# facebookresearch/co-tracker

Hardware: NVIDIA B200
Metric: tracked points*frames/sec at N=6400, T=16, 512^2 (higher is better)
Workload: dtype transformer + corr_mlp.fc2 + input_transform: bf16x3; correlation einsum: fp16x2; corr_mlp.fc1: bf16x3; fp32 accumulate, fp32 softmax/LayerNorm/GELU

## Files before the change

### cotracker_b200/csrc/api.cu

```cuda
#include <stdio.h>
#include <string.h>

#include <atomic>
#include <string>
#include <vector>

#include "../../include/ct3_b200.h"
#include "gemm.cuh"
#include "kernels.cuh"

using namespace ct3;

namespace {

thread_local char g_err[512] = "";
struct OptDef { const char* name; int lo, hi; };
enum { OPT_GEMM = 0, OPT_CORR, OPT_ATTN, OPT_PREC_CORR, OPT_PREC_FC1, OPT_FUSE, OPT_COUNT };
constexpr int kDefPrecCorr = 2, kDefPrecFc1 = 3;
constexpr OptDef kOptDefs[OPT_COUNT] = {
    {"gemm", 0, 1},
    {"corr", 0, 3},
    {"attn", 0, 2},
    {"prec.corr", 1, 3},
    {"prec.fc1", 1, 3},
    {"fuse", 0, 2},
};
thread_local int g_opt[OPT_COUNT] = {0, 0, 0, kDefPrecCorr, kDefPrecFc1, 1};
#define g_opt_gemm g_opt[OPT_GEMM]
#define g_opt_corr g_opt[OPT_CORR]
#define g_opt_attn g_opt[OPT_ATTN]

int fail(int code, const char* fmt, const char* detail = "") {
  snprintf(g_err, sizeof(g_err), fmt, detail);
  return code;
}
int fail_cuda(cudaError_t e, const char* where) {
  snprintf(g_err, sizeof(g_err), "%s: %s", where, cudaGetErrorString(e));
  return CT3_ECUDA;
}
#define CK(call, where)                                  \
  do {                                                   \
    cudaError_t e__ = (call);                            \
    if (e__ != cudaSuccess) return fail_cuda(e__, where); \
  } while (0)

int num_sms() {
  static std::atomic<int> cache[64] = {};
  int dev = 0;
  if (cudaGetDevice(&dev) != cudaSuccess) return 148;
  if (dev >= 0 && dev < 64) {
    const int c = cache[dev].load(std::memory_order_relaxed);
    if (c > 0) return c;
  }
  int n = 0;
  if (cudaDeviceGetAttribute(&n, cudaDevAttrMultiProcessorCount, dev) != cudaSuccess || n <= 0) n = 148;
  if (dev >= 0 && dev < 64) cache[dev].store(n, std::memory_order_relaxed);
  return n;
}


enum { CAT_CORR = 0, CAT_GEMM = 1, CAT_ATTN = 2, CAT_LN = 3, CAT_MISC = 4, CAT_ENC = 5, CAT_QKVA = 6, CAT_COUNT = 7 };
struct ProfRec { int cat; cudaEvent_t a, b; double flops; int launches; };
thread_local bool g_prof_on = false;
thread_local std::vector<ProfRec> g_prof;
struct ProfScope {
  cudaStream_t s; int cat; double flops; int launches; cudaEvent_t a = nullptr, b = nullptr;
  ProfScope(cudaStream_t s_, int cat_, double flops_ = 0.0, int launches_ = 1)
      : s(s_), cat(cat_), flops(flops_), launches(launches_) {
    if (g_prof_on && cat_ >= 0) { cudaEventCreate(&a); cudaEventCreate(&b); cudaEventRecord(a, s); }
  }
  ~ProfScope() {
    if (a) { cudaEventRecord(b, s); g_prof.push_back({cat, a, b, flops, launches}); }
  }
};

size_t align_up(size_t x, size_t a = 256) { return (x + a - 1) / a * a; }

struct Lin {
  size_t w = 0, b = 0;
  size_t ws = 0;
  int N = 0, K = 0, Kpad = 0;
};
struct Block {
  Lin qkv_h;
  Lin q;
  Lin kv;
  Lin kv_f;
  Lin out, fc1, fc2;
  size_t ctx_g = 0, ctx_b = 0;
  bool cross = false;
};
struct Layout {
  Lin corr_fc1, corr_fc2, in_tr;
  Lin corr_fc1_h;
  Lin corr_fc1_t, corr_fc1_th;
  Block time[kDepth], vself[kDepth], p2v[kDepth], v2p[kDepth];
  size_t heads_w = 0, heads_b = 0, virt = 0, win_f32 = 0;
  size_t scratch = 0;
  size_t total = 0;
};

int pad64(int k) { return (k + 63) / 64 * 64; }

void place_lin(Lin& l, int N, int K, size_t& off) {
  l.N = N;
  l.K = K;
  l.Kpad = pad64(K);
  l.w = off;
  off = align_up(off + (size_t)N * 2 * l.Kpad * sizeof(__nv_bfloat16));
  l.b = off;
// ... 88 lines not shown
  float* att_part;
  __nv_bfloat16* pyr_split;
  size_t total;
};
Workspace carve(void* base, int T, int N, int H4 = 0, int W4 = 0) {
  Workspace w;
  const size_t R = (size_t)(N + kV) * T, Rp = (size_t)N * T, Rv = (size_t)kV * T, Mc = Rp * kL;
  uint8_t* p = reinterpret_cast<uint8_t*>(base);
  size_t off = 0;
  auto take = [&](size_t bytes) { uint8_t* r = p + off; off = align_up(off + bytes, 1024); return r; };
  w.vol = (__nv_bfloat16*)take(Mc * 2 * kVolPad * 2);
  w.h1 = (__nv_bfloat16*)take(Mc * 2 * kCorrHid * 2);
  w.xs = (__nv_bfloat16*)take(Rp * 2 * kXPad * 2);
  w.tokens = (float*)take(R * kC * 4);
  w.traw = (__nv_bfloat16*)take(R * 2 * kC * 2);
  w.tstat = (float*)take(R * kLnParts * 2 * 4);
  w.ln = (__nv_bfloat16*)take(R * 2 * kC * 2);
  w.att = (__nv_bfloat16*)take(R * 2 * kC * 2);
  w.qkv = (float*)take(R * 3 * kC * 4);
  w.vqkv = (float*)take(Rv * 3 * kC * 4);
  w.hmid = (__nv_bfloat16*)take(R * 2 * kMlpHid * 2);
  w.row_bias = (float*)take((size_t)T * kC * 4);
  w.att_part = (float*)take(attention_partial_bytes(T, kV, kAttnMaxSplits));
  w.pyr_split = nullptr;
  if (H4 > 0 && W4 > 0 && corr_patch_supported(T, H4, W4))
    w.pyr_split = (__nv_bfloat16*)take((size_t)pyramid_layout(T, H4, W4).total * 4);
  w.total = off;
  return w;
}

struct Runner {
  const uint8_t* pk;
  const Layout& L;
  cudaStream_t s;
  int impl;
  const char* gerr = nullptr;

  int gemm(const __nv_bfloat16* x, const Lin& lin, int M, const GemmEpilogue& e, int products = 3, int fp16 = 0,
           int64_t x_ld = 0) {
    GemmProblem p;
    p.products = products;
    p.fp16 = fp16;
    p.x_ld = x_ld;
    p.x_split = x;
    p.w_split = reinterpret_cast<const __nv_bfloat16*>(pk + lin.w);
    p.M = M;
    p.N = lin.N;
    p.Kpad = lin.Kpad;
    p.epi = e;
    if (!p.epi.bias) p.epi.bias = reinterpret_cast<const float*>(pk + lin.b);
    if (M == 0) return 0;
    ProfScope ps(s, CAT_GEMM, 2.0 * (double)M * lin.N * lin.K);
    return gemm_launch(p, impl, num_sms(), s, &gerr);
  }
  static GemmEpilogue to_f32(float* out, int ld, bool residual) {
    GemmEpilogue e;
    e.out_f32 = out; e.ld_f32 = ld; e.residual = residual ? 1 : 0;
    return e;
  }
  static GemmEpilogue to_split(__nv_bfloat16* out, int ld, int lo_off, int act) {
    GemmEpilogue e;
    e.out_split = out; e.ld_split = ld; e.lo_off = lo_off; e.act = act;
    return e;
  }
};

#define RUNC(cat, call)                                                                  \
  do {                                                                                   \
    int rc__;                                                                            \
    { ProfScope ps__(R.s, cat); rc__ = (int)(call); }                                    \
    if (rc__ != 0) {                                                                     \
      snprintf(g_err, sizeof(g_err), "%s failed: %s (%s)", #call,                        \
               cudaGetErrorString((cudaError_t)rc__), R.gerr ? R.gerr : "");             \
      return CT3_ECUDA;                                                                  \
    }                                                                                    \
  } while (0)

int run_attention(Runner& R, const Workspace& W, const AttnParams& a, bool per_warp) {
  if (g_opt_attn == 1) return (int)launch_attention(a, R.s);
  if (g_opt_attn == 0 && !per_warp && a.Lq > kV && attention_p2v_supported(a)) return (int)launch_attention_p2v(a, R.s);
  return (int)launch_attention_tc(a, per_warp, W.att_part, num_sms(), R.s);
}

int mlp_half(Runner& R, const Workspace& W, const Block& b, int64_t row0, int rows) {
  float* x = W.tokens + row0 * kC;
  __nv_bfloat16* ln = W.ln + row0 * 2 * kC;
  __nv_bfloat16* hm = W.hmid + row0 * 2 * kMlpHid;
  RUNC(CAT_LN, launch_layernorm_split(x, rows, nullptr, nullptr, 1e-6f, ln, R.s));
  RUNC(-1, R.gemm(ln, b.fc1, rows, Runner::to_split(hm, 2 * kMlpHid, kMlpHid,  2)));
  RUNC(-1, R.gemm(hm, b.fc2, rows, Runner::to_f32(x, kC, true)));
  return 0;
}

int transformer_body(Runner& R, const Workspace& W, int T, int N) {
  const Layout& L = R.L;
  const int Rp = N * T, Rv = kV * T, Rall = Rp + Rv;
  const float scale = 1.0f / sqrtf((float)kDh);
  const uint8_t* pk = R.pk;
  RUNC(CAT_MISC, launch_init_virtual(W.tokens, reinterpret_cast<const float*>(pk + L.virt), T, N, R.s));
  float* vtok = W.tokens + (int64_t)Rp * kC;
  __nv_bfloat16* ln_p = W.ln;
  __nv_bfloat16* ln_v = W.ln + (int64_t)Rp * 2 * kC;
  __nv_bfloat16* att_p = W.att;
  __nv_bfloat16* att_v = W.att + (int64_t)Rp * 2 * kC;

  for (int i = 0; i < kDepth; ++i) {
    {
      const Block& b = L.time[i];
      RUNC(CAT_LN, launch_layernorm_split(W.tokens, Rall, nullptr, nullptr, 1e-6f, W.ln, R.s));
      if (g_opt[OPT_FUSE] >= 1 && R.impl == 0 && g_opt_attn != 1 && qkv_time_attn_supported(T)) {
        ProfScope ps(R.s, CAT_QKVA, 0.0);
        int rc = gemm_qkv_time_attn_launch(W.ln, reinterpret_cast<const __nv_bfloat16*>(pk + b.qkv_h.w),
                                           reinterpret_cast<const float*>(pk + b.qkv_h.b), Rall, kC, T, W.att, 2 * kC,
                                           kC, scale, nullptr, nullptr, 0.f, num_sms(), R.s, &R.gerr);
        if (rc != 0) {
          snprintf(g_err, sizeof(g_err), "fused qkv + time attention failed: %s (%s)",
                   cudaGetErrorString((cudaError_t)rc), R.gerr ? R.gerr : "");
          return CT3_ECUDA;
        }
      } else {
        RUNC(-1, R.gemm(W.ln, b.q, Rall, Runner::to_f32(W.qkv, 3 * kC, false)));
        AttnParams a{};
        a.q = W.qkv; a.q_ld = 3 * kC; a.q_col = 0;
        a.kv = W.qkv; a.kv_ld = 3 * kC; a.k_col = kC; a.v_col = 2 * kC;
        a.out = W.att; a.out_ld = 2 * kC; a.lo_off = kC;
        a.num_seq = N + kV; a.Lq = T; a.Lk = T;
        a.q_seq_stride = T; a.q_tok_stride = 1; a.k_seq_stride = T; a.k_tok_stride = 1;
        a.scale = scale;
        RUNC(CAT_ATTN, run_attention(R, W, a, true));
      }
      RUNC(-1, R.gemm(W.att, b.out, Rall, Runner::to_f32(W.tokens, kC, true)));
      if (int rc = mlp_half(R, W, b, 0, Rall)) return rc;
    }
    {
      const Block& b = L.v2p[i];
      RUNC(CAT_LN, launch_layernorm_split(vtok, Rv, nullptr, nullptr, 1e-6f, ln_v, R.s));
      RUNC(CAT_LN, launch_layernorm_split(W.tokens, Rp, reinterpret_cast<const float*>(pk + b.ctx_g),
                                 reinterpret_cast<const float*>(pk + b.ctx_b), 1e-5f, ln_p, R.s));
      RUNC(-1, R.gemm(ln_v, b.q, Rv, Runner::to_f32(W.vqkv, kC, false)));
      RUNC(-1, R.gemm(ln_p, b.kv, Rp, Runner::to_f32(W.qkv, 2 * kC, false)));
      AttnParams a{};
      a.q = W.vqkv; a.q_ld = kC; a.q_col = 0;
      a.kv = W.qkv; a.kv_ld = 2 * kC; a.k_col = 0; a.v_col = kC;
      a.out = att_v; a.out_ld = 2 * kC; a.lo_off = kC;
      a.num_seq = T; a.Lq = kV; a.Lk = N;
      a.q_seq_stride = 1; a.q_tok_stride = T; a.k_seq_stride = 1; a.k_tok_stride = T;
      a.scale = scale;
      RUNC(CAT_ATTN, run_attention(R, W, a, false));
      RUNC(-1, R.gemm(att_v, b.out, Rv, Runner::to_f32(vtok, kC, true)));
      if (int rc = mlp_half(R, W, b, Rp, Rv)) return rc;
    }
    {
      const Block& b = L.vself[i];
      RUNC(CAT_LN, launch_layernorm_split(vtok, Rv, nullptr, nullptr, 1e-6f, ln_v, R.s));
      RUNC(-1, R.gemm(ln_v, b.q, Rv, Runner::to_f32(W.vqkv, 3 * kC, false)));
      AttnParams a{};
      a.q = W.vqkv; a.q_ld = 3 * kC; a.q_col = 0;
      a.kv = W.vqkv; a.kv_ld = 3 * kC; a.k_col = kC; a.v_col = 2 * kC;
      a.out = att_v; a.out_ld = 2 * kC; a.lo_off = kC;
      a.num_seq = T; a.Lq = kV; a.Lk = kV;
      a.q_seq_stride = 1; a.q_tok_stride = T; a.k_seq_stride = 1; a.k_tok_stride = T;
      a.scale = scale;
      RUNC(CAT_ATTN, run_attention(R, W, a, false));
      RUNC(-1, R.gemm(att_v, b.out, Rv, Runner::to_f32(vtok, kC, true)));
      if (int rc = mlp_half(R, W, b, Rp, Rv)) return rc;
    }
    {
      const Block& b = L.p2v[i];
      RUNC(CAT_LN, launch_layernorm_split(W.tokens, Rp, nullptr, nullptr, 1e-6f, ln_p, R.s));
      RUNC(CAT_LN, launch_layernorm_split(vtok, Rv, reinterpret_cast<const float*>(pk + b.ctx_g),
                                 reinterpret_cast<const float*>(pk + b.ctx_b), 1e-5f, ln_v, R.s));
// ... 838 lines not shown
```

### cotracker_b200/csrc/common.cuh

```cuda
#pragma once
#include <cuda.h>
#include <cuda_bf16.h>
#include <cuda_fp16.h>
#include <cuda_runtime.h>
#include <stdint.h>

#include <atomic>

namespace ct3 {

struct DeviceOnce { std::atomic<uint64_t> done[2] = {}; };
template <typename F>
inline cudaError_t once_per_device(DeviceOnce& flag, F&& f) {
  int dev = 0;
  cudaError_t e = cudaGetDevice(&dev);
  if (e != cudaSuccess) return e;
  if (dev < 0 || dev >= 128) return f();
  const uint64_t bit = 1ull << (dev & 63);
  if (flag.done[dev >> 6].load(std::memory_order_acquire) & bit) return cudaSuccess;
  e = f();
  if (e == cudaSuccess) flag.done[dev >> 6].fetch_or(bit, std::memory_order_release);
  return e;
}

// ... 245 lines not shown
  asm volatile("tcgen05.dealloc.cta_group::1.sync.aligned.b32 %0, %1;" ::"r"(taddr), "r"(ncols) : "memory");
}
__device__ __forceinline__ uint64_t umma_desc_sw128(uint32_t smem_addr) {
  uint64_t d = 0;
  d |= (uint64_t)((smem_addr & 0x3FFFFu) >> 4);
  d |= (uint64_t)1 << 16;
  d |= (uint64_t)(1024 >> 4) << 32;
  d |= (uint64_t)1 << 46;
  d |= (uint64_t)2 << 61;
  return d;
}
__host__ __device__ constexpr uint32_t umma_idesc_bf16(int M, int N) {
  return (1u << 4) | (1u << 7) | (1u << 10) | ((uint32_t)(N >> 3) << 17) | ((uint32_t)(M >> 4) << 24);
}
__host__ __device__ constexpr uint32_t umma_idesc_16(int M, int N, bool fp16) {
  return (1u << 4) | (fp16 ? 0u : ((1u << 7) | (1u << 10))) | ((uint32_t)(N >> 3) << 17) | ((uint32_t)(M >> 4) << 24);
}
__device__ __forceinline__ void umma_bf16(uint32_t d_tmem, uint64_t adesc, uint64_t bdesc, uint32_t idesc,
                                          uint32_t accumulate) {
  asm volatile(
      "{\n\t"
      ".reg .pred p;\n\t"
      "setp.ne.b32 p, %4, 0;\n\t"
      "tcgen05.mma.cta_group::1.kind::f16 [%0], %1, %2, %3, p;\n\t"
      "}" ::"r"(d_tmem),
      "l"(adesc), "l"(bdesc), "r"(idesc), "r"(accumulate)
      : "memory");
}
__device__ __forceinline__ void umma_commit(uint64_t* bar) {
  asm volatile("tcgen05.commit.cta_group::1.mbarrier::arrive::one.shared::cluster.b64 [%0];" ::"r"(smem_u32(bar))
               : "memory");
}
__device__ __forceinline__ void umma_commit_mc(uint64_t* bar, uint16_t mask) {
  asm volatile(
      "tcgen05.commit.cta_group::1.mbarrier::arrive::one.shared::cluster.multicast::cluster.b64 [%0], %1;" ::"r"(
          smem_u32(bar)),
      "h"(mask)
      : "memory");
}
constexpr uint32_t kPeerBitMask = 0xFEFFFFFFu;
__device__ __forceinline__ void tmem_alloc_2sm(uint32_t* dst_smem, uint32_t ncols) {
  asm volatile("tcgen05.alloc.cta_group::2.sync.aligned.shared::cta.b32 [%0], %1;" ::"r"(smem_u32(dst_smem)),
               "r"(ncols)
               : "memory");
  asm volatile("tcgen05.relinquish_alloc_permit.cta_group::2.sync.aligned;" ::: "memory");
}
__device__ __forceinline__ void tmem_dealloc_2sm(uint32_t taddr, uint32_t ncols) {
  asm volatile("tcgen05.dealloc.cta_group::2.sync.aligned.b32 %0, %1;" ::"r"(taddr), "r"(ncols) : "memory");
}
__device__ __forceinline__ void tma_load_2d_2sm(void* smem_dst, const CUtensorMap* m, int c0, int c1, uint64_t* bar) {
  asm volatile(
      "cp.async.bulk.tensor.2d.cta_group::2.shared::cluster.global.mbarrier::complete_tx::bytes [%0], [%1, {%3, %4}], [%2];"
      ::"r"(smem_u32(smem_dst)), "l"(reinterpret_cast<uint64_t>(m)), "r"(smem_u32(bar) & kPeerBitMask), "r"(c0), "r"(c1)
      : "memory");
}
__device__ __forceinline__ void umma_bf16_2sm(uint32_t d_tmem, uint64_t adesc, uint64_t bdesc, uint32_t idesc,
                                              uint32_t accumulate) {
  asm volatile(
      "{\n\t"
      ".reg .pred p;\n\t"
      "setp.ne.b32 p, %4, 0;\n\t"
      "tcgen05.mma.cta_group::2.kind::f16 [%0], %1, %2, %3, p;\n\t"
      "}" ::"r"(d_tmem),
      "l"(adesc), "l"(bdesc), "r"(idesc), "r"(accumulate)
      : "memory");
}
__device__ __forceinline__ void umma_commit_2sm(uint64_t* bar) {
  asm volatile(
      "tcgen05.commit.cta_group::2.mbarrier::arrive::one.shared::cluster.multicast::cluster.b64 [%0], %1;" ::"r"(
          smem_u32(bar)),
      "h"((uint16_t)3)
      : "memory");
}
__device__ __forceinline__ void mbar_arrive_remote(uint64_t* bar, uint32_t cta) {
  asm volatile(
      "{\n\t"
      ".reg .b32 ra;\n\t"
      "mapa.shared::cluster.u32 ra, %0, %1;\n\t"
      "mbarrier.arrive.shared::cluster.b64 _, [ra];\n\t"
      "}" ::"r"(smem_u32(bar)),
      "r"(cta)
      : "memory");
}
__device__ __forceinline__ void tmem_ld32(uint32_t taddr, float (&v)[32]) {
  uint32_t r[32];
  asm volatile(
      "tcgen05.ld.sync.aligned.32x32b.x32.b32 "
      "{%0, %1, %2, %3, %4, %5, %6, %7, %8, %9, %10, %11, %12, %13, %14, %15, "
      "%16, %17, %18, %19, %20, %21, %22, %23, %24, %25, %26, %27, %28, %29, %30, %31}, [%32];"
      : "=r"(r[0]), "=r"(r[1]), "=r"(r[2]), "=r"(r[3]), "=r"(r[4]), "=r"(r[5]), "=r"(r[6]), "=r"(r[7]),
        "=r"(r[8]), "=r"(r[9]), "=r"(r[10]), "=r"(r[11]), "=r"(r[12]), "=r"(r[13]), "=r"(r[14]), "=r"(r[15]),
        "=r"(r[16]), "=r"(r[17]), "=r"(r[18]), "=r"(r[19]), "=r"(r[20]), "=r"(r[21]), "=r"(r[22]), "=r"(r[23]),
        "=r"(r[24]), "=r"(r[25]), "=r"(r[26]), "=r"(r[27]), "=r"(r[28]), "=r"(r[29]), "=r"(r[30]), "=r"(r[31])
      : "r"(taddr)
      : "memory");
  asm volatile("tcgen05.wait::ld.sync.aligned;" : "+r"(r[0]), "+r"(r[1]), "+r"(r[2]), "+r"(r[3]), "+r"(r[4]), "+r"(r[5]), "+r"(r[6]), "+r"(r[7]), "+r"(r[8]), "+r"(r[9]), "+r"(r[10]), "+r"(r[11]), "+r"(r[12]), "+r"(r[13]), "+r"(r[14]), "+r"(r[15]), "+r"(r[16]), "+r"(r[17]), "+r"(r[18]), "+r"(r[19]), "+r"(r[20]), "+r"(r[21]), "+r"(r[22]), "+r"(r[23]), "+r"(r[24]), "+r"(r[25]), "+r"(r[26]), "+r"(r[27]), "+r"(r[28]), "+r"(r[29]), "+r"(r[30]), "+r"(r[31]) :: "memory");
#pragma unroll
  for (int i = 0; i < 32; ++i) v[i] = __uint_as_float(r[i]);
}

__device__ __forceinline__ void tmem_ld8_nowait(uint32_t taddr, uint32_t (&r)[8]) {
  asm volatile(
      "tcgen05.ld.sync.aligned.32x32b.x8.b32 {%0, %1, %2, %3, %4, %5, %6, %7}, [%8];"
      : "=r"(r[0]), "=r"(r[1]), "=r"(r[2]), "=r"(r[3]), "=r"(r[4]), "=r"(r[5]), "=r"(r[6]), "=r"(r[7])
      : "r"(taddr)
      : "memory");
}
__device__ __forceinline__ void tmem_ld_wait() { asm volatile("tcgen05.wait::ld.sync.aligned;" ::: "memory"); }
__device__ __forceinline__ void tmem_ld_wait8(uint32_t (&r)[8]) {
  asm volatile("tcgen05.wait::ld.sync.aligned;"
               : "+r"(r[0]), "+r"(r[1]), "+r"(r[2]), "+r"(r[3]), "+r"(r[4]), "+r"(r[5]), "+r"(r[6]), "+r"(r[7])
               ::"memory");
}

__device__ __forceinline__ void tmem_ld64(uint32_t taddr, float (&v)[64]) {
  uint32_t r[64];
  asm volatile(
      "tcgen05.ld.sync.aligned.32x32b.x64.b32 "
      "{%0, %1, %2, %3, %4, %5, %6, %7, %8, %9, %10, %11, %12, %13, %14, %15, %16, %17, %18, %19, %20, %21, %22, %23, %24, %25, %26, %27, %28, %29, %30, %31, %32, %33, %34, %35, %36, %37, %38, %39, %40, %41, %42, %43, %44, %45, %46, %47, %48, %49, %50, %51, %52, %53, %54, %55, %56, %57, %58, %59, %60, %61, %62, %63}, [%64];"
      : "=r"(r[0]), "=r"(r[1]), "=r"(r[2]), "=r"(r[3]), "=r"(r[4]), "=r"(r[5]), "=r"(r[6]), "=r"(r[7]), "=r"(r[8]), "=r"(r[9]), "=r"(r[10]), "=r"(r[11]), "=r"(r[12]), "=r"(r[13]), "=r"(r[14]), "=r"(r[15]), "=r"(r[16]), "=r"(r[17]), "=r"(r[18]), "=r"(r[19]), "=r"(r[20]), "=r"(r[21]), "=r"(r[22]), "=r"(r[23]), "=r"(r[24]), "=r"(r[25]), "=r"(r[26]), "=r"(r[27]), "=r"(r[28]), "=r"(r[29]), "=r"(r[30]), "=r"(r[31]), "=r"(r[32]), "=r"(r[33]), "=r"(r[34]), "=r"(r[35]), "=r"(r[36]), "=r"(r[37]), "=r"(r[38]), "=r"(r[39]), "=r"(r[40]), "=r"(r[41]), "=r"(r[42]), "=r"(r[43]), "=r"(r[44]), "=r"(r[45]), "=r"(r[46]), "=r"(r[47]), "=r"(r[48]), "=r"(r[49]), "=r"(r[50]), "=r"(r[51]), "=r"(r[52]), "=r"(r[53]), "=r"(r[54]), "=r"(r[55]), "=r"(r[56]), "=r"(r[57]), "=r"(r[58]), "=r"(r[59]), "=r"(r[60]), "=r"(r[61]), "=r"(r[62]), "=r"(r[63])
      : "r"(taddr)
      : "memory");
  asm volatile("tcgen05.wait::ld.sync.aligned;"
               : "+r"(r[0]), "+r"(r[1]), "+r"(r[2]), "+r"(r[3]), "+r"(r[4]), "+r"(r[5]), "+r"(r[6]), "+r"(r[7]), "+r"(r[8]), "+r"(r[9]), "+r"(r[10]), "+r"(r[11]), "+r"(r[12]), "+r"(r[13]), "+r"(r[14]), "+r"(r[15]), "+r"(r[16]), "+r"(r[17]), "+r"(r[18]), "+r"(r[19]), "+r"(r[20]), "+r"(r[21]), "+r"(r[22]), "+r"(r[23]), "+r"(r[24]), "+r"(r[25]), "+r"(r[26]), "+r"(r[27]), "+r"(r[28]), "+r"(r[29]), "+r"(r[30]), "+r"(r[31]), "+r"(r[32]), "+r"(r[33]), "+r"(r[34]), "+r"(r[35]), "+r"(r[36]), "+r"(r[37]), "+r"(r[38]), "+r"(r[39]), "+r"(r[40]), "+r"(r[41]), "+r"(r[42]), "+r"(r[43]), "+r"(r[44]), "+r"(r[45]), "+r"(r[46]), "+r"(r[47]), "+r"(r[48]), "+r"(r[49]), "+r"(r[50]), "+r"(r[51]), "+r"(r[52]), "+r"(r[53]), "+r"(r[54]), "+r"(r[55]), "+r"(r[56]), "+r"(r[57]), "+r"(r[58]), "+r"(r[59]), "+r"(r[60]), "+r"(r[61]), "+r"(r[62]), "+r"(r[63])
               ::"memory");
#pragma unroll
  for (int i = 0; i < 64; ++i) v[i] = __uint_as_float(r[i]);
}

__device__ __forceinline__ void tmem_ld16(uint32_t taddr, float (&v)[16]) {
  uint32_t r[16];
  asm volatile(
      "tcgen05.ld.sync.aligned.32x32b.x16.b32 "
      "{%0, %1, %2, %3, %4, %5, %6, %7, %8, %9, %10, %11, %12, %13, %14, %15}, [%16];"
      : "=r"(r[0]), "=r"(r[1]), "=r"(r[2]), "=r"(r[3]), "=r"(r[4]), "=r"(r[5]), "=r"(r[6]), "=r"(r[7]),
        "=r"(r[8]), "=r"(r[9]), "=r"(r[10]), "=r"(r[11]), "=r"(r[12]), "=r"(r[13]), "=r"(r[14]), "=r"(r[15])
      : "r"(taddr)
      : "memory");
  asm volatile("tcgen05.wait::ld.sync.aligned;"
               : "+r"(r[0]), "+r"(r[1]), "+r"(r[2]), "+r"(r[3]), "+r"(r[4]), "+r"(r[5]), "+r"(r[6]), "+r"(r[7]),
                 "+r"(r[8]), "+r"(r[9]), "+r"(r[10]), "+r"(r[11]), "+r"(r[12]), "+r"(r[13]), "+r"(r[14]), "+r"(r[15])
               ::"memory");
#pragma unroll
  for (int i = 0; i < 16; ++i) v[i] = __uint_as_float(r[i]);
}

}
```

### cotracker_b200/csrc/gemm.cu

```cuda
#include "gemm.cuh"

namespace ct3 {
namespace {

constexpr int BM = 128, BN = 128, BK = 64;
constexpr int ACC = 2;
constexpr int TILE_A = BM * BK * 2;
constexpr int TILE_B = BN * BK * 2;
constexpr int EPI_WARPS = 16;
constexpr int CW = 16;
constexpr int STG_WORDS = 32 * CW;
constexpr int MAX_STAGES = 6;
template <int NPROD>
struct Cfg {
  static constexpr int AP = NPROD >= 3 ? 2 : 1;
  static constexpr int BP = NPROD >= 2 ? 2 : 1;
  static constexpr int STAGE_BYTES = AP * TILE_A + BP * TILE_B;
  static constexpr int STAGES = NPROD >= 3 ? 3 : (NPROD == 2 ? 4 : 6);
  static constexpr int OFF_B = AP * TILE_A;
};
constexpr int OFF_STG = 3 * 65536;
static_assert(Cfg<1>::STAGES * Cfg<1>::STAGE_BYTES == OFF_STG && Cfg<2>::STAGES * Cfg<2>::STAGE_BYTES == OFF_STG &&
              Cfg<3>::STAGES * Cfg<3>::STAGE_BYTES == OFF_STG && Cfg<4>::STAGES * Cfg<4>::STAGE_BYTES == OFF_STG &&
              Cfg<5>::STAGES * Cfg<5>::STAGE_BYTES == OFF_STG, "ring size");
// ... 303 lines not shown
        for (int kb = 0; kb < num_kb; ++kb) {
          mbar_wait(&empty_bar[stage], phase ^ 1u);
          if (rank == 0) mbar_arrive_expect_tx(&full_bar[stage], TX_BYTES);
          uint8_t* s = smem + stage * STAGE_BYTES;
          tma_load_2d_2sm(s, &tmX, kb * BK, mt * BM, &full_bar[stage]);
          if (C::AP == 2) tma_load_2d_2sm(s + TILE_A, &tmX, Kpad + kb * BK, mt * BM, &full_bar[stage]);
          tma_load_2d_2sm(s + C::OFF_B, &tmW, kb * BK, wrow, &full_bar[stage]);
          if (C::BP == 2) tma_load_2d_2sm(s + C::OFF_B + TILE_B, &tmW, Kpad + kb * BK, wrow, &full_bar[stage]);
          if (++stage == STAGES) { stage = 0; phase ^= 1u; }
        }
      }
    }
  } else if (warp == 1) {
    if (rank == 0 && elect_one()) {
      const uint32_t idesc = umma_idesc_16(256, BNP, fp16 != 0);
      int stage = 0, acc = 0;
      uint32_t phase = 0, acc_phase = 0;
      for (int tile = first; tile < num_tiles; tile += step) {
        mbar_wait(&tempty_bar[acc], acc_phase ^ 1u);
        tc_fence_after_sync();
        const uint32_t d_tmem = tmem_base + (uint32_t)(acc * BNP);
        for (int kb = 0; kb < num_kb; ++kb) {
          mbar_wait(&full_bar[stage], phase);
          tc_fence_after_sync();
          const uint32_t s = smem_u32(smem + stage * STAGE_BYTES);
          const uint32_t a_hi = s, a_lo = s + TILE_A, b_hi = s + C::OFF_B, b_lo = b_hi + TILE_B;
#pragma unroll
          for (int kk = 0; kk < BK / 16; ++kk) {
            const uint32_t koff = kk * 32;
            const uint64_t dah = umma_desc_sw128(a_hi + koff), dbh = umma_desc_sw128(b_hi + koff);
            const uint32_t first = (kb | kk) != 0 ? 1u : 0u;
            if (NPROD >= 3) {
              umma_bf16_2sm(d_tmem, umma_desc_sw128(a_lo + koff), dbh, idesc, first);
              umma_bf16_2sm(d_tmem, dah, umma_desc_sw128(b_lo + koff), idesc, 1u);
              umma_bf16_2sm(d_tmem, dah, dbh, idesc, 1u);
            } else if (NPROD == 2) {
              umma_bf16_2sm(d_tmem, dah, umma_desc_sw128(b_lo + koff), idesc, first);
              umma_bf16_2sm(d_tmem, dah, dbh, idesc, 1u);
            } else {
              umma_bf16_2sm(d_tmem, dah, dbh, idesc, first);
            }
          }
          umma_commit_2sm(&empty_bar[stage]);
          if (++stage == STAGES) { stage = 0; phase ^= 1u; }
        }
        umma_commit_2sm(&tfull_bar[acc]);
        if (++acc == ACC) { acc = 0; acc_phase ^= 1u; }
      }
    }
  } else {
    const int quarter = warp & 3;
    constexpr int CH = BNP / CW / (EPI_WARPS / 4);
    const int chunk0 = ((warp - 2) >> 2) * CH;
    int acc = 0;
    uint32_t acc_phase = 0;
    for (int tile = first; tile < num_tiles; tile += step) {
      const int mt = (tile / num_nt) * 2 + (int)rank, nt = tile % num_nt;
      mbar_wait(&tfull_bar[acc], acc_phase);
      tc_fence_after_sync();
      const int row0 = mt * BM + quarter * 32;
      uint32_t* stg = reinterpret_cast<uint32_t*>(smem + OFF_STG) + (warp - 2) * STG_WORDS;
      float ln_mean = 0.f, ln_rstd = 1.f;
      if constexpr (NPROD == 5) {
        if (row0 + lane < M) ln_row_stats(epi.ln_part + (int64_t)(row0 + lane) * kLnParts * 2, epi.ln_eps, ln_mean, ln_rstd);
      }
#pragma unroll 1
      for (int chunk = chunk0; chunk < chunk0 + CH; ++chunk) {
        float v[CW];
        const uint32_t taddr = tmem_base + ((uint32_t)(quarter * 32) << 16) + (uint32_t)(acc * BNP + chunk * CW);
        tmem_ld16(taddr, v);
        epilogue_chunk<NPROD == 4, NPROD == 5>(epi, M, N, row0, nt * BNP + chunk * CW, lane, v, stg, ln_mean, ln_rstd);
      }
      tc_fence_before_sync();
      __syncwarp();
      if (lane == 0) mbar_arrive_remote(&tempty_bar[acc], 0);
      if (++acc == ACC) { acc = 0; acc_phase ^= 1u; }
    }
  }

  tc_fence_before_sync();
  __syncthreads();
  cluster_sync_all();
  if (warp == 1) tmem_dealloc_2sm(tmem_base, TCOLS);
}

namespace qa {
constexpr int BNQ = 144;
constexpr int TILE_BQ = (BNQ / 2) * BK * 2;
constexpr int STAGE = 2 * TILE_A + 2 * TILE_BQ;
constexpr int NSTAGE = 2;
constexpr int KV_LD = 100;
constexpr int KV_BYTES = BM * KV_LD * 4;
constexpr int OFF_KV = NSTAGE * STAGE;
constexpr int OFF_BARQ = OFF_KV + 2 * KV_BYTES;
constexpr int SMEM = OFF_BARQ + 256 + 1024;
constexpr int EPIW = 8;
constexpr int NTHREADS = (2 + EPIW) * 32;
constexpr int ACC_STRIDE = 256;
static_assert(SMEM <= 232448, "shared memory budget");
}

__global__ void __launch_bounds__(qa::NTHREADS, 1)
gemm_qkv_time_attn_kernel(const __grid_constant__ CUtensorMap tmX, const __grid_constant__ CUtensorMap tmW, int M,
                          int Kpad, int T, int R, float scale_log2e, GemmEpilogue epi) {
  using namespace qa;
  constexpr uint32_t TX_BYTES = 2u * (2u * TILE_A + 2u * TILE_BQ);
  extern __shared__ __align__(1024) uint8_t smem_raw[];
  uint8_t* smem = smem_align1024(smem_raw);
  uint64_t* full_bar = reinterpret_cast<uint64_t*>(smem + OFF_BARQ);
  uint64_t* empty_bar = full_bar + NSTAGE;
  uint64_t* tfull_bar = empty_bar + NSTAGE;
  uint64_t* tempty_bar = tfull_bar + ACC;
  uint32_t* tmem_slot = reinterpret_cast<uint32_t*>(tempty_bar + ACC);
  float* kvs = reinterpret_cast<float*>(smem + OFF_KV);

  const int warp = threadIdx.x >> 5, lane = threadIdx.x & 31;
  const uint32_t rank = cluster_ctarank();
  if (warp == 0 && lane == 0) {
    tma_prefetch_desc(&tmX);
    tma_prefetch_desc(&tmW);
    for (int i = 0; i < NSTAGE; ++i) {
      mbar_init(&full_bar[i], 1);
      mbar_init(&empty_bar[i], 1);
    }
    for (int i = 0; i < ACC; ++i) {
      mbar_init(&tfull_bar[i], 1);
      mbar_init(&tempty_bar[i], 2 * 4);
    }
    fence_barrier_init();
  }
  if (warp == 1) tmem_alloc_2sm(tmem_slot, 512);
  tc_fence_before_sync();
  __syncthreads();
  cluster_sync_all();
  tc_fence_after_sync();
  const uint32_t tmem_base = *tmem_slot;

  const int num_mt = (M + R - 1) / R;
  const int num_mp = (num_mt + 1) / 2;
  const int num_tiles = num_mp * kHeads;
  const int num_kb = Kpad / BK;
  const int first = blockIdx.x >> 1, step = gridDim.x >> 1;

  if (warp == 0) {
    if (elect_one()) {
      int stage = 0;
      uint32_t phase = 0;
      for (int tile = first; tile < num_tiles; tile += step) {
        const int mt = (tile / kHeads) * 2 + (int)rank, h = tile % kHeads;
        const int wrow = h * BNQ + (int)rank * (BNQ / 2);
        for (int kb = 0; kb < num_kb; ++kb) {
          mbar_wait(&empty_bar[stage], phase ^ 1u);
          if (rank == 0) mbar_arrive_expect_tx(&full_bar[stage], TX_BYTES);
          uint8_t* s = smem + stage * STAGE;
          tma_load_2d_2sm(s, &tmX, kb * BK, mt * R, &full_bar[stage]);
          tma_load_2d_2sm(s + TILE_A, &tmX, Kpad + kb * BK, mt * R, &full_bar[stage]);
          tma_load_2d_2sm(s + 2 * TILE_A, &tmW, kb * BK, wrow, &full_bar[stage]);
          tma_load_2d_2sm(s + 2 * TILE_A + TILE_BQ, &tmW, Kpad + kb * BK, wrow, &full_bar[stage]);
          if (++stage == NSTAGE) { stage = 0; phase ^= 1u; }
        }
      }
    }
  } else if (warp == 1) {
    if (rank == 0 && elect_one()) {
      constexpr uint32_t idesc = umma_idesc_bf16(256, BNQ);
      int stage = 0, acc = 0;
// ... 286 lines not shown
  }
  const int groups = ((num_mt + 1) / 2) * (p.N / bnp);
  int pairs = num_sms / 2;
  if (pairs > groups) pairs = groups;
  cudaLaunchConfig_t cfg = {};
  cfg.gridDim = dim3(2 * pairs);
  cfg.blockDim = dim3(THREADS);
  cfg.dynamicSmemBytes = SMEM_BYTES;
  cfg.stream = stream;
  cudaLaunchAttribute at[1];
  at[0].id = cudaLaunchAttributeClusterDimension;
  at[0].val.clusterDim.x = 2;
  at[0].val.clusterDim.y = 1;
  at[0].val.clusterDim.z = 1;
  cfg.attrs = at;
  cfg.numAttrs = 1;
  cudaError_t e = (bnp == 256)
      ? cudaLaunchKernelEx(&cfg, gemm_split3_pair_kernel<256, NPROD>, tmX, tmW, p.M, p.N, p.Kpad, p.fp16, p.epi)
      : cudaLaunchKernelEx(&cfg, gemm_split3_pair_kernel<192, NPROD>, tmX, tmW, p.M, p.N, p.Kpad, p.fp16, p.epi);
  if (e != cudaSuccess) return e;
  return cudaGetLastError();
}

}

bool qkv_time_attn_supported(int T) { return T >= 1 && T <= BM; }

int gemm_qkv_time_attn_launch(const __nv_bfloat16* x_split, const __nv_bfloat16* w_heads, const float* bias_heads,
                              int M, int Kpad, int T, __nv_bfloat16* att_split, int64_t ld_split, int lo_off,
                              float scale, const float* ln_part, const float* ln_wsum, float ln_eps, int num_sms,
                              cudaStream_t stream, const char** err) {
  *err = nullptr;
  if (M <= 0 || Kpad <= 0 || (Kpad % BK) != 0 || !qkv_time_attn_supported(T) || (M % T) != 0) {
    *err = "qkv_time_attn: need M > 0, M % T == 0, 1 <= T <= 128, Kpad % 64 == 0";
    return (int)cudaErrorInvalidValue;
  }
  if (((reinterpret_cast<uintptr_t>(x_split) | reinterpret_cast<uintptr_t>(w_heads) |
        reinterpret_cast<uintptr_t>(att_split)) & 15) || (ld_split % 8) != 0 || (lo_off % 8) != 0) {
    *err = "qkv_time_attn: operands must be 16-byte aligned";
    return (int)cudaErrorInvalidValue;
  }
  const int R = (BM / T) * T;
  CUtensorMap tmX, tmW;
  if (!make_tmap(&tmX, x_split, (uint64_t)M, 2ull * Kpad) ||
      !make_tmap(&tmW, w_heads, (uint64_t)(kHeads * qa::BNQ), 2ull * Kpad, (uint32_t)(qa::BNQ / 2))) {
    *err = "qkv_time_attn: cuTensorMapEncodeTiled failed";
    return (int)cudaErrorInvalidValue;
  }
  static DeviceOnce attr;
  cudaError_t e = once_per_device(attr, [&] {
    return cudaFuncSetAttribute(gemm_qkv_time_attn_kernel, cudaFuncAttributeMaxDynamicSharedMemorySize, qa::SMEM);
  });
  if (e != cudaSuccess) { *err = "qkv_time_attn: cudaFuncSetAttribute failed"; return (int)e; }
  const int num_mt = (M + R - 1) / R;
  const int groups = ((num_mt + 1) / 2) * kHeads;
  int pairs = num_sms / 2;
  if (pairs > groups) pairs = groups;
  GemmEpilogue epi;
  epi.bias = bias_heads;
  epi.out_split = att_split;
  epi.ld_split = ld_split;
  epi.lo_off = lo_off;
  epi.ln_part = ln_part;
  epi.ln_wsum = ln_wsum;
  epi.ln_eps = ln_eps;
  cudaLaunchConfig_t cfg = {};
  cfg.gridDim = dim3(2 * pairs);
  cfg.blockDim = dim3(qa::NTHREADS);
  cfg.dynamicSmemBytes = qa::SMEM;
  cfg.stream = stream;
  cudaLaunchAttribute at[1];
  at[0].id = cudaLaunchAttributeClusterDimension;
  at[0].val.clusterDim.x = 2;
  at[0].val.clusterDim.y = 1;
  at[0].val.clusterDim.z = 1;
  cfg.attrs = at;
  cfg.numAttrs = 1;
  e = cudaLaunchKernelEx(&cfg, gemm_qkv_time_attn_kernel, tmX, tmW, M, Kpad, T, R,
                         scale * 1.44269504088896340736f, epi);
  if (e != cudaSuccess) return (int)e;
  return (int)cudaGetLastError();
}

int gemm_launch(const GemmProblem& p, int impl, int num_sms, cudaStream_t stream, const char** err) {
  *err = nullptr;
  if (p.M <= 0 || p.N <= 0 || p.Kpad <= 0 || (p.N % BN) != 0 || (p.Kpad % BK) != 0) {
    *err = "gemm: need M>0, N % 128 == 0, Kpad % 64 == 0";
    return (int)cudaErrorInvalidValue;
  }
  if (p.products < 1 || p.products > 3) {
    *err = "gemm: products must be 1, 2 or 3";
    return (int)cudaErrorInvalidValue;
  }
  const int64_t x_ld = p.x_ld ? p.x_ld : 2 * (int64_t)p.Kpad;
  if (x_ld < (p.products == 3 ? 2 : 1) * (int64_t)p.Kpad || (x_ld % 8) != 0) {
    *err = "gemm: x_ld too small for the operand planes this product count reads";
    return (int)cudaErrorInvalidValue;
  }
  if ((reinterpret_cast<uintptr_t>(p.x_split) | reinterpret_cast<uintptr_t>(p.w_split)) & 15) {
    *err = "gemm: operands must be 16-byte aligned";
    return (int)cudaErrorInvalidValue;
  }
  if (p.epi.raw_split && (p.N != kLnDim || !p.epi.out_f32 || !p.epi.stat_part || impl == 1)) {
    *err = "gemm: raw_split/stat_part need the fp32 output path of the tensor-core kernels with N == 384";
    return (int)cudaErrorInvalidValue;
  }
  if (p.epi.ln_part && !p.epi.ln_wsum) {
    *err = "gemm: ln_part needs ln_wsum";
    return (int)cudaErrorInvalidValue;
  }
  if (impl == 1) {
    dim3 grid((p.N + 63) / 64, (p.M + 63) / 64);
    gemm_split3_simt_kernel<<<grid, 256, 0, stream>>>(p.x_split, p.w_split, p.M, p.N, p.Kpad, x_ld, p.products,
                                                      p.fp16, p.epi);
    return (int)cudaGetLastError();
  }
  const int num_mt = (p.M + BM - 1) / BM;
  int bnp = 0;
  if (impl == 0 && num_mt >= 2 * num_sms) bnp = (p.N % 256 == 0) ? 256 : ((p.N % 192 == 0) ? 192 : 0);
  CUtensorMap tmX, tmW;
  if (!make_tmap(&tmX, p.x_split, (uint64_t)p.M, (uint64_t)x_ld) ||
      !make_tmap(&tmW, p.w_split, (uint64_t)p.N, 2ull * p.Kpad, bnp ? (uint32_t)(bnp / 2) : 128u)) {
    *err = "gemm: cuTensorMapEncodeTiled failed";
    return (int)cudaErrorInvalidValue;
  }
  static DeviceOnce attr_set;
  {
    cudaError_t e = once_per_device(attr_set, [&] {
      cudaError_t e = set_attrs<3>();
      if (e == cudaSuccess) e = set_attrs<4>();
      if (e == cudaSuccess) e = set_attrs<5>();
      if (e == cudaSuccess) e = set_attrs<2>();
      if (e == cudaSuccess) e = set_attrs<1>();
      return e;
    });
    if (e != cudaSuccess) { *err = "gemm: cudaFuncSetAttribute(max dynamic smem) failed"; return (int)e; }
  }
  if (p.epi.ln_part && (p.products != 3 || p.epi.raw_split)) {
    *err = "gemm: the LayerNorm-consumer epilogue needs 3 products and cannot be combined with raw_split";
    return (int)cudaErrorInvalidValue;
  }
  cudaError_t e = (p.products == 3 && p.epi.raw_split) ? launch_tc<4>(p, tmX, tmW, bnp, num_mt, num_sms, stream)
                : (p.products == 3 && p.epi.ln_part) ? launch_tc<5>(p, tmX, tmW, bnp, num_mt, num_sms, stream)
                : p.products == 3 ? launch_tc<3>(p, tmX, tmW, bnp, num_mt, num_sms, stream)
                : p.products == 2 ? launch_tc<2>(p, tmX, tmW, bnp, num_mt, num_sms, stream)
                                  : launch_tc<1>(p, tmX, tmW, bnp, num_mt, num_sms, stream);
  return (int)e;
}

}
```

### cotracker_b200/csrc/gemm.cuh

```cuda
#pragma once
#include "common.cuh"

namespace ct3 {

struct GemmEpilogue {
  const float* bias = nullptr;
  const float* row_bias = nullptr;
  int row_mod = 1;
  int act = 0;
  float* out_f32 = nullptr;
  int64_t ld_f32 = 0;
  int residual = 0;
  __nv_bfloat16* out_split = nullptr;
  int64_t ld_split = 0;
  int lo_off = 0;
  int row_group = 1;
  const float* ln_part = nullptr;
  const float* ln_wsum = nullptr;
  float ln_eps = 0.f;
  __nv_bfloat16* raw_split = nullptr;
  float* stat_part = nullptr;
};
constexpr int kLnDim = 384;
constexpr int kLnParts = kLnDim / 16;

struct GemmProblem {
  const __nv_bfloat16* x_split;
  const __nv_bfloat16* w_split;
  int M, N, Kpad;
  int products = 3;
  int fp16 = 0;
  int64_t x_ld = 0;
  GemmEpilogue epi;
};

bool encode_tensor_map(CUtensorMap* m, CUtensorMapDataType dtype, int rank, const void* base, const uint64_t* dims,
                       const uint64_t* strides_bytes, const uint32_t* box, CUtensorMapSwizzle swizzle);

int gemm_launch(const GemmProblem& p, int impl, int num_sms, cudaStream_t stream, const char** err);

bool qkv_time_attn_supported(int T);
int gemm_qkv_time_attn_launch(const __nv_bfloat16* x_split, const __nv_bfloat16* w_heads, const float* bias_heads,
                              int M, int Kpad, int T, __nv_bfloat16* att_split, int64_t ld_split, int lo_off,
                              float scale, const float* ln_part, const float* ln_wsum, float ln_eps, int num_sms,
                              cudaStream_t stream, const char** err);

__device__ __forceinline__ void ln_row_stats(const float* part, float eps, float& mean, float& rstd) {
  float s = 0.f, ss = 0.f;
#pragma unroll
  for (int i = 0; i < kLnParts; ++i) {
    const float2 p = __ldg(reinterpret_cast<const float2*>(part) + i);
    s += p.x;
    ss += p.y;
  }
  mean = s * (1.0f / kLnDim);
  const float var = fmaxf(ss * (1.0f / kLnDim) - mean * mean, 0.f);
  rstd = rsqrtf(var + eps);
}

}
```

Before: 1.195 million.

## Fuse transformer MLP fc1, GELU and fc2 into one 2-SM tcgen05 kernel

Adds a persistent 2-CTA cluster kernel that computes fc1 per 128-wide hidden chunk into TMEM, applies bias, GELU and a bf16 hi/lo split into shared memory, then feeds that chunk directly into the fc2 accumulation with the residual epilogue. This removes the round trip of the 1536-wide hidden activation through global memory and one kernel launch per MLP. It is on by default when there are enough row tiles to fill the SMs, and costs a more complex pipeline whose GEMM1/GEMM2 alternation may serialise tensor-core work and add register pressure.

```diff
diff --git a/cotracker_b200/csrc/api.cu b/cotracker_b200/csrc/api.cu
--- a/cotracker_b200/csrc/api.cu
+++ b/cotracker_b200/csrc/api.cu
@@ -15,7 +15,7 @@
 
 thread_local char g_err[512] = "";
 struct OptDef { const char* name; int lo, hi; };
-enum { OPT_GEMM = 0, OPT_CORR, OPT_ATTN, OPT_PREC_CORR, OPT_PREC_FC1, OPT_FUSE, OPT_COUNT };
+enum { OPT_GEMM = 0, OPT_CORR, OPT_ATTN, OPT_PREC_CORR, OPT_PREC_FC1, OPT_FUSE, OPT_MLP, OPT_COUNT };
 constexpr int kDefPrecCorr = 2, kDefPrecFc1 = 3;
 constexpr OptDef kOptDefs[OPT_COUNT] = {
     {"gemm", 0, 1},
@@ -24,8 +24,9 @@
     {"prec.corr", 1, 3},
     {"prec.fc1", 1, 3},
     {"fuse", 0, 2},
+    {"mlp", 0, 2},
 };
-thread_local int g_opt[OPT_COUNT] = {0, 0, 0, kDefPrecCorr, kDefPrecFc1, 1};
+thread_local int g_opt[OPT_COUNT] = {0, 0, 0, kDefPrecCorr, kDefPrecFc1, 1, 1};
 #define g_opt_gemm g_opt[OPT_GEMM]
 #define g_opt_corr g_opt[OPT_CORR]
 #define g_opt_attn g_opt[OPT_ATTN]
@@ -280,11 +281,30 @@
   return (int)launch_attention_tc(a, per_warp, W.att_part, num_sms(), R.s);
 }
 
+bool mlp_fused(const Runner& R, int rows) {
+  if (R.impl != 0 || g_opt[OPT_MLP] == 0) return false;
+  return g_opt[OPT_MLP] == 2 || mlp_pair_tiles(rows) >= 4 * (num_sms() / 2);
+}
+
 int mlp_half(Runner& R, const Workspace& W, const Block& b, int64_t row0, int rows) {
   float* x = W.tokens + row0 * kC;
   __nv_bfloat16* ln = W.ln + row0 * 2 * kC;
   __nv_bfloat16* hm = W.hmid + row0 * 2 * kMlpHid;
   RUNC(CAT_LN, launch_layernorm_split(x, rows, nullptr, nullptr, 1e-6f, ln, R.s));
+  if (mlp_fused(R, rows)) {
+    const uint8_t* pk = R.pk;
+    ProfScope ps(R.s, CAT_GEMM, 2.0 * 2.0 * (double)rows * kC * kMlpHid);
+    int rc = mlp_split3_pair_launch(ln, reinterpret_cast<const __nv_bfloat16*>(pk + b.fc1.w),
+                                    reinterpret_cast<const float*>(pk + b.fc1.b),
+                                    reinterpret_cast<const __nv_bfloat16*>(pk + b.fc2.w),
+                                    reinterpret_cast<const float*>(pk + b.fc2.b), x, rows, num_sms(), R.s, &R.gerr);
+    if (rc != 0) {
+      snprintf(g_err, sizeof(g_err), "fused MLP failed: %s (%s)", cudaGetErrorString((cudaError_t)rc),
+               R.gerr ? R.gerr : "");
+      return CT3_ECUDA;
+    }
+    return 0;
+  }
   RUNC(-1, R.gemm(ln, b.fc1, rows, Runner::to_split(hm, 2 * kMlpHid, kMlpHid,  2)));
   RUNC(-1, R.gemm(hm, b.fc2, rows, Runner::to_f32(x, kC, true)));
   return 0;
diff --git a/cotracker_b200/csrc/common.cuh b/cotracker_b200/csrc/common.cuh
--- a/cotracker_b200/csrc/common.cuh
+++ b/cotracker_b200/csrc/common.cuh
@@ -351,6 +351,16 @@
       "r"(cta)
       : "memory");
 }
+__device__ __forceinline__ void mbar_arrive_remote_release(uint64_t* bar, uint32_t cta) {
+  asm volatile(
+      "{\n\t"
+      ".reg .b32 ra;\n\t"
+      "mapa.shared::cluster.u32 ra, %0, %1;\n\t"
+      "mbarrier.arrive.release.cluster.shared::cluster.b64 _, [ra];\n\t"
+      "}" ::"r"(smem_u32(bar)),
+      "r"(cta)
+      : "memory");
+}
 __device__ __forceinline__ void tmem_ld32(uint32_t taddr, float (&v)[32]) {
   uint32_t r[32];
   asm volatile(
diff --git a/cotracker_b200/csrc/gemm.cu b/cotracker_b200/csrc/gemm.cu
--- a/cotracker_b200/csrc/gemm.cu
+++ b/cotracker_b200/csrc/gemm.cu
@@ -409,6 +409,250 @@
   __syncthreads();
   cluster_sync_all();
   if (warp == 1) tmem_dealloc_2sm(tmem_base, TCOLS);
+}
+
+namespace mlp {
+constexpr int HC = 128;
+constexpr int NCH = kMlpHid / HC;
+constexpr int KB1 = kC / BK;
+constexpr int KB2 = HC / BK;
+constexpr int N2 = 192;
+constexpr int W1H = (HC / 2) * BK * 2;
+constexpr int W2H = (N2 / 2) * BK * 2;
+constexpr int STAGE = 2 * TILE_A + 2 * W1H;
+static_assert(STAGE == 4 * W2H, "G1 and G2 stages have the same size");
+constexpr int NSTAGE = 3;
+constexpr int HS_TILE = BM * BK * 2;
+constexpr int OFF_HS = NSTAGE * STAGE;
+constexpr int OFF_BARM = OFF_HS + 2 * KB2 * HS_TILE;
+constexpr int SMEM = OFF_BARM + 256 + 1024;
+constexpr uint32_t TX_BYTES = 2u * STAGE;
+constexpr uint32_t H_COL = kC;
+static_assert(SMEM <= 232448, "shared memory budget");
+static_assert(EPI_WARPS * STG_WORDS * 4 <= 2 * KB2 * HS_TILE, "output staging fits in Hs");
+}
+
+__global__ void __launch_bounds__(THREADS, 1)
+mlp_split3_pair_kernel(const __grid_constant__ CUtensorMap tmX, const __grid_constant__ CUtensorMap tmW1,
+                       const __grid_constant__ CUtensorMap tmW2, int M, const float* __restrict__ b1,
+                       GemmEpilogue epi) {
+  using namespace mlp;
+  extern __shared__ __align__(1024) uint8_t smem_raw[];
+  uint8_t* smem = smem_align1024(smem_raw);
+  uint8_t* hs = smem + OFF_HS;
+  uint64_t* full_bar = reinterpret_cast<uint64_t*>(smem + OFF_BARM);
+  uint64_t* empty_bar = full_bar + NSTAGE;
+  uint64_t* h_full = empty_bar + NSTAGE;
+  uint64_t* h_empty = h_full + 1;
+  uint64_t* hs_full = h_empty + 1;
+  uint64_t* hs_empty = hs_full + 1;
+  uint64_t* o_full = hs_empty + 1;
+  uint64_t* o_empty = o_full + 1;
+  uint32_t* tmem_slot = reinterpret_cast<uint32_t*>(o_empty + 1);
+
+  const int warp = threadIdx.x >> 5, lane = threadIdx.x & 31;
+  const uint32_t rank = cluster_ctarank();
+  if (warp == 0 && lane == 0) {
+    tma_prefetch_desc(&tmX);
+    tma_prefetch_desc(&tmW1);
+    tma_prefetch_desc(&tmW2);
+    for (int i = 0; i < NSTAGE; ++i) {
+      mbar_init(&full_bar[i], 1);
+      mbar_init(&empty_bar[i], 1);
+    }
+    mbar_init(h_full, 1);
+    mbar_init(h_empty, 2 * EPI_WARPS);
+    mbar_init(hs_full, 2 * EPI_WARPS);
+    mbar_init(hs_empty, 1);
+    mbar_init(o_full, 1);
+    mbar_init(o_empty, 2 * EPI_WARPS);
+    fence_barrier_init();
+  }
+  if (warp == 1) tmem_alloc_2sm(tmem_slot, 512);
+  tc_fence_before_sync();
+  __syncthreads();
+  cluster_sync_all();
+  tc_fence_after_sync();
+  const uint32_t tmem_base = *tmem_slot;
+
+  const int num_tiles = ((M + BM - 1) / BM + 1) / 2;
+  const int first = blockIdx.x >> 1, step = gridDim.x >> 1;
+  const int total = first < num_tiles ? ((num_tiles - 1 - first) / step + 1) * NCH : 0;
+
+  if (warp == 0) {
+    if (elect_one()) {
+      int stage = 0;
+      uint32_t phase = 0;
+      auto acquire = [&]() -> uint8_t* {
+        mbar_wait(&empty_bar[stage], phase ^ 1u);
+        if (rank == 0) mbar_arrive_expect_tx(&full_bar[stage], TX_BYTES);
+        return smem + stage * STAGE;
+      };
+      auto advance = [&]() { if (++stage == NSTAGE) { stage = 0; phase ^= 1u; } };
+      auto load_g1 = [&](int g) {
+        const int mt = (first + (g / NCH) * step) * 2 + (int)rank;
+        const int wrow = (g % NCH) * HC + (int)rank * (HC / 2);
+        for (int kb = 0; kb < KB1; ++kb) {
+          uint8_t* s = acquire();
+          tma_load_2d_2sm(s, &tmX, kb * BK, mt * BM, &full_bar[stage]);
+          tma_load_2d_2sm(s + TILE_A, &tmX, kC + kb * BK, mt * BM, &full_bar[stage]);
+          tma_load_2d_2sm(s + 2 * TILE_A, &tmW1, kb * BK, wrow, &full_bar[stage]);
+          tma_load_2d_2sm(s + 2 * TILE_A + W1H, &tmW1, kC + kb * BK, wrow, &full_bar[stage]);
+          advance();
+        }
+      };
+      auto load_g2 = [&](int g) {
+        for (int kb = 0; kb < KB2; ++kb) {
+          uint8_t* s = acquire();
+          const int k = (g % NCH) * HC + kb * BK;
+#pragma unroll
+          for (int n = 0; n < 2; ++n) {
+            const int wrow = n * N2 + (int)rank * (N2 / 2);
+            tma_load_2d_2sm(s + (2 * n) * W2H, &tmW2, k, wrow, &full_bar[stage]);
+            tma_load_2d_2sm(s + (2 * n + 1) * W2H, &tmW2, kMlpHid + k, wrow, &full_bar[stage]);
+          }
+          advance();
+        }
+      };
+      if (total > 0) load_g1(0);
+      for (int g = 0; g < total; ++g) {
+        if (g + 1 < total) load_g1(g + 1);
+        load_g2(g);
+      }
+    }
+  } else if (warp == 1) {
+    if (rank == 0 && elect_one()) {
+      constexpr uint32_t idesc1 = umma_idesc_bf16(256, HC), idesc2 = umma_idesc_bf16(256, N2);
+      int stage = 0;
+      uint32_t phase = 0, h_phase = 0, hs_phase = 0, o_phase = 0;
+      auto mma_g1 = [&]() {
+        mbar_wait(h_empty, h_phase ^ 1u);
+        tc_fence_after_sync();
+        const uint32_t d_tmem = tmem_base + H_COL;
+        for (int kb = 0; kb < KB1; ++kb) {
+          mbar_wait(&full_bar[stage], phase);
+          tc_fence_after_sync();
+          const uint32_t s = smem_u32(smem + stage * STAGE);
+          const uint32_t a_hi = s, a_lo = s + TILE_A, b_hi = s + 2 * TILE_A, b_lo = b_hi + W1H;
+#pragma unroll
+          for (int kk = 0; kk < BK / 16; ++kk) {
+            const uint32_t koff = kk * 32;
+            const uint64_t dah = umma_desc_sw128(a_hi + koff), dbh = umma_desc_sw128(b_hi + koff);
+            umma_bf16_2sm(d_tmem, umma_desc_sw128(a_lo + koff), dbh, idesc1, (kb | kk) != 0 ? 1u : 0u);
+            umma_bf16_2sm(d_tmem, dah, umma_desc_sw128(b_lo + koff), idesc1, 1u);
+            umma_bf16_2sm(d_tmem, dah, dbh, idesc1, 1u);
+          }
+          umma_commit_2sm(&empty_bar[stage]);
+          if (++stage == NSTAGE) { stage = 0; phase ^= 1u; }
+        }
+        umma_commit_2sm(h_full);
+        h_phase ^= 1u;
+      };
+      auto mma_g2 = [&](int c) {
+        if (c == 0) {
+          mbar_wait(o_empty, o_phase ^ 1u);
+          tc_fence_after_sync();
+        }
+        mbar_wait(hs_full, hs_phase);
+        tc_fence_after_sync();
+        const uint32_t h = smem_u32(hs);
+        for (int kb = 0; kb < KB2; ++kb) {
+          mbar_wait(&full_bar[stage], phase);
+          tc_fence_after_sync();
+          const uint32_t s = smem_u32(smem + stage * STAGE);
+          const uint32_t a_hi = h + (2 * kb) * HS_TILE, a_lo = a_hi + HS_TILE;
+#pragma unroll
+          for (int kk = 0; kk < BK / 16; ++kk) {
+            const uint32_t koff = kk * 32;
+            const uint32_t acc = (c | kb | kk) != 0 ? 1u : 0u;
+            const uint64_t dah = umma_desc_sw128(a_hi + koff), dal = umma_desc_sw128(a_lo + koff);
+#pragma unroll
+            for (int n = 0; n < 2; ++n) {
+              const uint32_t d_tmem = tmem_base + (uint32_t)(n * N2);
+              const uint32_t b_hi = s + (2 * n) * W2H, b_lo = b_hi + W2H;
+              const uint64_t dbh = umma_desc_sw128(b_hi + koff);
+              umma_bf16_2sm(d_tmem, dal, dbh, idesc2, acc);
+              umma_bf16_2sm(d_tmem, dah, umma_desc_sw128(b_lo + koff), idesc2, 1u);
+              umma_bf16_2sm(d_tmem, dah, dbh, idesc2, 1u);
+            }
+          }
+          umma_commit_2sm(&empty_bar[stage]);
+          if (++stage == NSTAGE) { stage = 0; phase ^= 1u; }
+        }
+        umma_commit_2sm(hs_empty);
+        hs_phase ^= 1u;
+        if (c == NCH - 1) { umma_commit_2sm(o_full); o_phase ^= 1u; }
+      };
+      if (total > 0) mma_g1();
+      for (int g = 0; g < total; ++g) {
+        if (g + 1 < total) mma_g1();
+        mma_g2(g % NCH);
+      }
+    }
+  } else {
+    const int quarter = warp & 3;
+    const int wg = (warp - 2) >> 2;
+    const int r = quarter * 32 + lane;
+    const uint32_t tlane = tmem_base + ((uint32_t)(quarter * 32) << 16);
+    const int hs_row = (2 * (wg >> 1)) * HS_TILE + r * 128;
+    const int j0 = (wg & 1) * 4;
+    uint32_t h_phase = 0, hs_phase = 0, o_phase = 0;
+    for (int g = 0; g < total; ++g) {
+      const int c = g % NCH;
+      mbar_wait(h_full, h_phase);
+      h_phase ^= 1u;
+      tc_fence_after_sync();
+      float v[32];
+      tmem_ld32(tlane + H_COL + (uint32_t)(wg * 32), v);
+      tc_fence_before_sync();
+      __syncwarp();
+      if (lane == 0) mbar_arrive_remote(h_empty, 0);
+      mbar_wait(hs_empty, hs_phase ^ 1u);
+      hs_phase ^= 1u;
+      const float4* b4 = reinterpret_cast<const float4*>(b1 + c * HC + wg * 32);
+#pragma unroll
+      for (int q = 0; q < 4; ++q) {
+        const float4 ba = __ldg(b4 + 2 * q), bb = __ldg(b4 + 2 * q + 1);
+        float* u = v + 8 * q;
+        u[0] += ba.x; u[1] += ba.y; u[2] += ba.z; u[3] += ba.w;
+        u[4] += bb.x; u[5] += bb.y; u[6] += bb.z; u[7] += bb.w;
+        uint32_t hi[4], lo[4];
+#pragma unroll
+        for (int i = 0; i < 4; ++i) split2(gelu_tanh(u[2 * i]), gelu_tanh(u[2 * i + 1]), hi[i], lo[i]);
+        const int j = ((j0 + q) ^ (r & 7)) * 16;
+        *reinterpret_cast<uint4*>(hs + hs_row + j) = make_uint4(hi[0], hi[1], hi[2], hi[3]);
+        *reinterpret_cast<uint4*>(hs + hs_row + HS_TILE + j) = make_uint4(lo[0], lo[1], lo[2], lo[3]);
+      }
+      fence_proxy_async_smem();
+      __syncwarp();
+      if (lane == 0) mbar_arrive_remote_release(hs_full, 0);
+      if (c == NCH - 1) {
+        const int mt = (first + (g / NCH) * step) * 2 + (int)rank;
+        mbar_wait(o_full, o_phase);
+        o_phase ^= 1u;
+        tc_fence_after_sync();
+        const int row0 = mt * BM + quarter * 32;
+        uint32_t* stg = reinterpret_cast<uint32_t*>(hs) + (warp - 2) * STG_WORDS;
+        constexpr int CH = kC / CW / (EPI_WARPS / 4);
+#pragma unroll 1
+        for (int ch = 0; ch < CH; ++ch) {
+          const int col0 = (wg * CH + ch) * CW;
+          float o[CW];
+          tmem_ld16(tlane + (uint32_t)col0, o);
+          epilogue_chunk<false, false>(epi, M, kC, row0, col0, lane, o, stg);
+        }
+        tc_fence_before_sync();
+        __syncwarp();
+        if (lane == 0) mbar_arrive_remote(o_empty, 0);
+        asm volatile("bar.sync 1, %0;" ::"n"(EPI_WARPS * 32) : "memory");
+      }
+    }
+  }
+
+  tc_fence_before_sync();
+  __syncthreads();
+  cluster_sync_all();
+  if (warp == 1) tmem_dealloc_2sm(tmem_base, 512);
 }
 
 namespace qa {
@@ -861,6 +1105,58 @@
   return (int)cudaGetLastError();
 }
 
+int mlp_pair_tiles(int M) { return ((M + BM - 1) / BM + 1) / 2; }
+
+int mlp_split3_pair_launch(const __nv_bfloat16* ln_split, const __nv_bfloat16* w1, const float* b1,
+                           const __nv_bfloat16* w2, const float* b2, float* tokens, int M, int num_sms,
+                           cudaStream_t stream, const char** err) {
+  *err = nullptr;
+  if (M <= 0) {
+    *err = "mlp: need M > 0";
+    return (int)cudaErrorInvalidValue;
+  }
+  if ((reinterpret_cast<uintptr_t>(ln_split) | reinterpret_cast<uintptr_t>(w1) | reinterpret_cast<uintptr_t>(w2) |
+       reinterpret_cast<uintptr_t>(b1) | reinterpret_cast<uintptr_t>(b2) | reinterpret_cast<uintptr_t>(tokens)) & 15) {
+    *err = "mlp: operands must be 16-byte aligned";
+    return (int)cudaErrorInvalidValue;
+  }
+  CUtensorMap tmX, tmW1, tmW2;
+  if (!make_tmap(&tmX, ln_split, (uint64_t)M, 2ull * kC) ||
+      !make_tmap(&tmW1, w1, (uint64_t)kMlpHid, 2ull * kC, (uint32_t)(mlp::HC / 2)) ||
+      !make_tmap(&tmW2, w2, (uint64_t)kC, 2ull * kMlpHid, (uint32_t)(mlp::N2 / 2))) {
+    *err = "mlp: cuTensorMapEncodeTiled failed";
+    return (int)cudaErrorInvalidValue;
+  }
+  static DeviceOnce attr;
+  cudaError_t e = once_per_device(attr, [&] {
+    return cudaFuncSetAttribute(mlp_split3_pair_kernel, cudaFuncAttributeMaxDynamicSharedMemorySize, mlp::SMEM);
+  });
+  if (e != cudaSuccess) { *err = "mlp: cudaFuncSetAttribute failed"; return (int)e; }
+  GemmEpilogue epi;
+  epi.bias = b2;
+  epi.out_f32 = tokens;
+  epi.ld_f32 = kC;
+  epi.residual = 1;
+  const int tiles = mlp_pair_tiles(M);
+  int pairs = num_sms / 2;
+  if (pairs > tiles) pairs = tiles;
+  cudaLaunchConfig_t cfg = {};
+  cfg.gridDim = dim3(2 * pairs);
+  cfg.blockDim = dim3(THREADS);
+  cfg.dynamicSmemBytes = mlp::SMEM;
+  cfg.stream = stream;
+  cudaLaunchAttribute at[1];
+  at[0].id = cudaLaunchAttributeClusterDimension;
+  at[0].val.clusterDim.x = 2;
+  at[0].val.clusterDim.y = 1;
+  at[0].val.clusterDim.z = 1;
+  cfg.attrs = at;
+  cfg.numAttrs = 1;
+  e = cudaLaunchKernelEx(&cfg, mlp_split3_pair_kernel, tmX, tmW1, tmW2, M, b1, epi);
+  if (e != cudaSuccess) return (int)e;
+  return (int)cudaGetLastError();
+}
+
 int gemm_launch(const GemmProblem& p, int impl, int num_sms, cudaStream_t stream, const char** err) {
   *err = nullptr;
   if (p.M <= 0 || p.N <= 0 || p.Kpad <= 0 || (p.N % BN) != 0 || (p.Kpad % BK) != 0) {
diff --git a/cotracker_b200/csrc/gemm.cuh b/cotracker_b200/csrc/gemm.cuh
--- a/cotracker_b200/csrc/gemm.cuh
+++ b/cotracker_b200/csrc/gemm.cuh
@@ -45,6 +45,11 @@
                               float scale, const float* ln_part, const float* ln_wsum, float ln_eps, int num_sms,
                               cudaStream_t stream, const char** err);
 
+int mlp_split3_pair_launch(const __nv_bfloat16* ln_split, const __nv_bfloat16* w1, const float* b1,
+                           const __nv_bfloat16* w2, const float* b2, float* tokens, int M, int num_sms,
+                           cudaStream_t stream, const char** err);
+int mlp_pair_tiles(int M);
+
 __device__ __forceinline__ void ln_row_stats(const float* part, float eps, float& mean, float& rstd) {
   float s = 0.f, ss = 0.f;
 #pragma unroll
```

Measured after the change: 1.227 million (median of 6 runs). +2.6%, better.
